# ajzhai/PEANUT

Hardware: AMD Instinct MI355X
Metric: maps/sec for 480x480x(4+N_cat) prediction fwd, batch 32 (higher is better)
Workload: dtype f32; 1 GPU; 480x480, 14-channel (4+10) partial maps -> 6-class prediction forward (PSPNet R50-V1c-D8), batch 32 per GPU, seeded random-init weights; survey_config=2, global_batch=32, parallelism=dp1 (map shards, no data-path collective)

## Files before the change

peanut_amd/csrc/conv_pw_ares.hip:

```cpp
#include <stdlib.h>

#include "common.h"
#include "conv_common.h"

namespace peanut {

namespace {

typedef const __attribute__((address_space(1))) void* gptr_t;
typedef __attribute__((address_space(3))) void* lptr_t;

__device__ __forceinline__ float load_uncounted(const float* ptr) {
  float v;
  asm volatile("global_load_dword %0, %1, off" : "=v"(v) : "v"(ptr) : "memory");
  return v;
}
template <int CH>
__device__ __forceinline__ void wait_uncounted(const float (&r)[CH], float a, float b) {
  static_assert(CH == 4 || CH == 8, "chunk of 4 or 8 values");
  __builtin_amdgcn_sched_barrier(0);
  if constexpr (CH == 4)
    asm volatile("s_waitcnt vmcnt(0)" ::"v"(r[0]), "v"(r[1]), "v"(r[2]), "v"(r[3]), "v"(a), "v"(b) : "memory");
  else
    asm volatile("s_waitcnt vmcnt(0)" ::"v"(r[0]), "v"(r[1]), "v"(r[2]), "v"(r[3]), "v"(r[4]), "v"(r[5]), "v"(r[6]), "v"(r[7]), "v"(a), "v"(b)
                 : "memory");
  __builtin_amdgcn_sched_barrier(0);
}

template <int NK, bool FLUSH>
__global__ __launch_bounds__(512) void conv_pw_ares_kernel(const ConvKParams p) {
  constexpr int BK = 32, K = NK * BK, TILE = 128 * BK;
  constexpr int CH = 32 / NK;
  static_assert(NK == 4 || NK == 8, "K = 128 or 256");
  __shared__ __attribute__((aligned(1024))) float smem[(NK + 2) * TILE];
  float* const bst = smem + NK * TILE;

  const int tid = threadIdx.x, lane = tid & 63;
  const int wave = __builtin_amdgcn_readfirstlane(tid >> 6);
  const int lr = lane >> 3, lp = lane & 7;
  const int wm = wave >> 2, wn = wave & 3;
  const int li = lane & 31, hi = lane >> 5;
  const bool late = p.phase_shift && wave >= 4;

  const int G = gridDim.x, bid = blockIdx.x;
  const int lw = (bid & 7) * (G >> 3) + (bid >> 3);
  const int NT = p.ntiles;
  const long long U = (long long)p.mtiles * NT;
  const int u0 = (int)(U * lw / G), u1 = (int)(U * (lw + 1) / G);
  if (u0 >= u1) return;

  const int pbn = p.ares_pbn;
  unsigned a_off[2], b_off[2];
#pragma unroll
  for (int j = 0; j < 2; ++j) {
    const int r = (wave * 2 + j) * 8 + lr;
    const int c = lp ^ ((r >> 1) & 7);
    a_off[j] = r * K + c * 4;
    b_off[j] = (r / pbn) * (NK * pbn * BK) + (r % pbn) * BK + c * 4;
  }
  auto dma_a = [&](int mt, int s) {
    const float* base = p.x + (size_t)mt * (128 * K) + s * BK;
#pragma unroll
    for (int j = 0; j < 2; ++j)
      __builtin_amdgcn_global_load_lds((gptr_t)(base + a_off[j]), (lptr_t)(smem + s * TILE + (wave * 2 + j) * 256), 16, 0, 0);
  };
  auto dma_b = [&](int mt, int nt, int kt, int stage) {
    const float* base = p.w + (p.mt_per_group ? (size_t)(mt / p.mt_per_group) * p.w_group_stride : 0) + (size_t)nt * (128 * K) + kt * (pbn * BK);
#pragma unroll
    for (int j = 0; j < 2; ++j)
      __builtin_amdgcn_global_load_lds((gptr_t)(base + b_off[j]), (lptr_t)(bst + stage * TILE + (wave * 2 + j) * 256), 16, 0, 0);
  };

  const int swz = (li >> 1) & 7;
  int sw[4];
#pragma unroll
  for (int ks = 0; ks < 4; ++ks) sw[ks] = ((ks * 2 + hi) ^ swz) * 4;
  const int a_row = (wm * 64 + li) * BK;
  const int b_row = (wn * 32 + li) * BK;

  f32x16 acc[2], acc2[2], prev[2];
#pragma unroll
  for (int t = 0; t < 2; ++t)
#pragma unroll
    for (int r = 0; r < 16; ++r) { acc[t][r] = 0.f; acc2[t][r] = 0.f; prev[t][r] = 0.f; }

  const size_t lane_el = (size_t)(wm * 64 + 4 * hi) * p.cout + wn * 32 + li;
  const bool has_res = p.res != nullptr;
  const size_t rstride = has_res ? (size_t)p.cout : 0;
  const size_t ostride = (size_t)p.cout;
  const float* res_run = has_res ? p.res + lane_el : p.zeros;
  float* out_run = p.y + lane_el;
  const float* prev_sc = p.scale + wn * 32 + li;
  const float* prev_sh = p.shift + wn * 32 + li;
  bool prev_valid = false;
  float scv = 1.f, shv = 0.f;
  const float alpha = p.alpha;
  const bool relu = p.relu != 0;

#define ARES_CHUNK_LOADS(kt)                                                              \
  float resv[CH];                                                                         \
  if ((kt) == 0) {                                                                        \
    scv = load_uncounted(prev_sc);                                                        \
    shv = load_uncounted(prev_sh);                                                        \
  }                                                                                       \
  _Pragma("unroll") for (int i = 0; i < CH; ++i)                                          \
    resv[i] = load_uncounted(res_run + (size_t)(8 * (i >> 2) + (i & 3)) * rstride);       \
  res_run += (size_t)(2 * CH) * rstride;
#define ARES_CHUNK_FINISH(kt)                                                             \
  if (prev_valid) {                                                   \
    _Pragma("unroll") for (int i = 0; i < CH; ++i) {                                      \
      const int idx = (kt) * CH + i;                                                      \
      float v = prev[idx >> 4][idx & 15] * (scv * alpha) + shv;                           \
      v += resv[i];                                                                       \
      if (relu) v = relu_keep_nan(v);                                                     \
      out_run[(size_t)(8 * (i >> 2) + (i & 3)) * ostride] = v;                            \
    }                                                                                     \
  }                                                                                       \
  out_run += (size_t)(2 * CH) * ostride;

  {
    const int mt = u0 / NT, nt = u0 - mt * NT;
#pragma unroll
    for (int s = 0; s < NK; ++s) dma_a(mt, s);
    dma_b(mt, nt, 0, 0);
    asm volatile("s_waitcnt vmcnt(0)" ::: "memory");
    __builtin_amdgcn_s_barrier();
    asm volatile("" ::: "memory");
  }

  int stage = 0;
  for (int u = u0; u < u1; ++u) {
    const int mt = u / NT, nt = u - mt * NT;
    const bool nxt = u + 1 < u1;
    const int mt_n = nxt ? (u + 1) / NT : mt;
    const int nt_n = nxt ? (u + 1) - mt_n * NT : 0;
    const bool refill_next = nxt && mt_n != mt;

    static_for<NK>([&](auto kc) {
      constexpr int kt = decltype(kc)::value;
      const float* const cur_b = bst + stage * TILE;
      const float* const cur_a = smem + kt * TILE;
      const bool more = (kt + 1 < NK) || nxt;
      ARES_CHUNK_LOADS(kt)
      auto request = [&]() {
        if (more) {
          if (kt + 1 < NK) dma_b(mt, nt, kt + 1, stage ^ 1);
          else dma_b(mt_n, nt_n, 0, stage ^ 1);
        }
      };
      if (!late) request();
      __builtin_amdgcn_sched_barrier(0);
      f32x4 af[4][2], bf[4];
#pragma unroll
      for (int j = 0; j < 4; ++j) {
        af[j][0] = *reinterpret_cast<const f32x4*>(cur_a + a_row + sw[j]);
        af[j][1] = *reinterpret_cast<const f32x4*>(cur_a + a_row + 32 * BK + sw[j]);
        bf[j] = *reinterpret_cast<const f32x4*>(cur_b + b_row + sw[j]);
      }
#pragma unroll
      for (int j = 0; j < 2; ++j)
#pragma unroll
        for (int kk = 0; kk < 4; ++kk)
#pragma unroll
          for (int t = 0; t < 2; ++t) acc[t] = __builtin_amdgcn_mfma_f32_32x32x2f32(af[j][t][kk], bf[j][kk], acc[t], 0, 0, 0);
      __builtin_amdgcn_sched_barrier(0);
      if (late) request();
      __builtin_amdgcn_sched_barrier(0);
#pragma unroll
      for (int j = 2; j < 4; ++j)
#pragma unroll
        for (int kk = 0; kk < 4; ++kk)
#pragma unroll
          for (int t = 0; t < 2; ++t) acc[t] = __builtin_amdgcn_mfma_f32_32x32x2f32(af[j][t][kk], bf[j][kk], acc[t], 0, 0, 0);
      if (FLUSH && (kt & 1)) {
#pragma unroll
        for (int t = 0; t < 2; ++t) {
          acc2[t] += acc[t];
#pragma unroll
          for (int r = 0; r < 16; ++r) acc[t][r] = 0.f;
        }
      }
      wait_uncounted<CH>(resv, scv, shv);
      ARES_CHUNK_FINISH(kt)
      if (kt >= 1) { if (refill_next) dma_a(mt_n, kt - 1); }
      asm volatile("s_waitcnt lgkmcnt(0)" ::: "memory");
      __builtin_amdgcn_s_barrier();
      asm volatile("" ::: "memory");
      stage ^= 1;
    });

#pragma unroll
    for (int t = 0; t < 2; ++t) {
      prev[t] = FLUSH ? acc2[t] : acc[t];
#pragma unroll
      for (int r = 0; r < 16; ++r) { acc[t][r] = 0.f; acc2[t][r] = 0.f; }
    }
    {
      const size_t unit_el = (size_t)mt * 128 * p.cout + (size_t)nt * 128 + lane_el;
      res_run = has_res ? p.res + unit_el : p.zeros;
      out_run = p.y + unit_el;
      const int ss_off = (p.mt_per_group && p.ss_group_stride) ? (mt / p.mt_per_group) * p.ss_group_stride : 0;
      prev_sc = p.scale + ss_off + nt * 128 + wn * 32 + li;
      prev_sh = p.shift + ss_off + nt * 128 + wn * 32 + li;
      prev_valid = true;
    }
    if (refill_next) dma_a(mt_n, NK - 1);
  }

  static_for<NK>([&](auto kc) {
    constexpr int kt = decltype(kc)::value;
    ARES_CHUNK_LOADS(kt)
    wait_uncounted<CH>(resv, scv, shv);
    ARES_CHUNK_FINISH(kt)
  });
#undef ARES_CHUNK_LOADS
#undef ARES_CHUNK_FINISH
}

template <int NK, bool FLUSH>
int launch_ares_t(ConvKParams p, hipStream_t stream) {
  const int cus = device_cus();
  if (cus < 8) return fail(-3, "conv_pw_ares: no current device");
  const long long U = (long long)p.mtiles * p.ntiles;
  long long G = U < cus ? U : cus;
  G -= G % 8;
  if (G < 8) return fail(-2, "conv_pw_ares: launch too small");
  hipLaunchKernelGGL((conv_pw_ares_kernel<NK, FLUSH>), dim3((unsigned)G), dim3(512), 0, stream, p);
  hipError_t e = hipGetLastError();
  if (e != hipSuccess) return fail(-3, std::string("conv_pw_ares launch: ") + hipGetErrorString(e));
  return 0;
}

}

bool conv_pw_uses_ares(int cin, int cout, long long M, int stride, bool two_source, int flush_ktiles, int bn_tile) {
  const bool on = opt(OPT_PW_ARES) != 0;
  const long long min_units = opt(OPT_PW_ARES_MINUNITS);
  if (!on || two_source || (cin != 128 && cin != 256) || stride != 1 || M % 128 != 0 || cout % 128 != 0) return false;
  if (bn_tile != 64 && bn_tile != 128) return false;
  if (flush_ktiles != 0 && flush_ktiles != 2) return false;
  return (M / 128) * (cout / 128) >= min_units;
}

int launch_conv_pw_ares(const ConvKParams& p0, int bn_tile, hipStream_t stream) {
  ConvKParams p = p0;
  p.phase_shift = opt(OPT_PW256_PHASE) != 0;
  p.ares_pbn = bn_tile;
  p.mtiles = p.M / 128;
  p.ntiles = p.cout / 128;
  const bool flush = p.flush == 2;
  if (p.c1 == 256) return flush ? launch_ares_t<8, true>(p, stream) : launch_ares_t<8, false>(p, stream);
  return flush ? launch_ares_t<4, true>(p, stream) : launch_ares_t<4, false>(p, stream);
}

}
```

Before: 888.1 maps/s.

## Defer epilogue stores by one chunk and use SGPR-base addressing in pointwise conv

The fused pointwise-conv epilogue now keeps each chunk's results in registers and issues their global stores during the next chunk's DMA request. The wait then lets those stores stay in flight (vmcnt(N)) instead of draining all memory ops before the barrier. Residual and output addressing switches to a scalar base plus a 32-bit per-lane offset to cut 64-bit address arithmetic, and the A-tile refill is issued earlier. The change also adds peeled first and second units, optional trace and ablation macros, and an s_nop before each load, which adds code complexity and may overflow 32-bit offsets on large tensors.

```diff
diff --git a/peanut_amd/csrc/conv_pw_ares.hip b/peanut_amd/csrc/conv_pw_ares.hip
--- a/peanut_amd/csrc/conv_pw_ares.hip
+++ b/peanut_amd/csrc/conv_pw_ares.hip
@@ -10,19 +10,21 @@
 typedef const __attribute__((address_space(1))) void* gptr_t;
 typedef __attribute__((address_space(3))) void* lptr_t;
 
-__device__ __forceinline__ float load_uncounted(const float* ptr) {
+__device__ __forceinline__ float load_uncounted(const float* base, unsigned byte_off) {
   float v;
-  asm volatile("global_load_dword %0, %1, off" : "=v"(v) : "v"(ptr) : "memory");
+  asm volatile("s_nop 4\n\tglobal_load_dword %0, %1, %2" : "=v"(v) : "v"(byte_off), "s"(base) : "memory");
   return v;
 }
-template <int CH>
+template <int CH, int N>
 __device__ __forceinline__ void wait_uncounted(const float (&r)[CH], float a, float b) {
   static_assert(CH == 4 || CH == 8, "chunk of 4 or 8 values");
+  static_assert(N == 0 || N == CH, "nothing, or the stores of one chunk");
   __builtin_amdgcn_sched_barrier(0);
   if constexpr (CH == 4)
-    asm volatile("s_waitcnt vmcnt(0)" ::"v"(r[0]), "v"(r[1]), "v"(r[2]), "v"(r[3]), "v"(a), "v"(b) : "memory");
+    asm volatile("s_waitcnt vmcnt(%0)" ::"n"(N), "v"(r[0]), "v"(r[1]), "v"(r[2]), "v"(r[3]), "v"(a), "v"(b) : "memory");
   else
-    asm volatile("s_waitcnt vmcnt(0)" ::"v"(r[0]), "v"(r[1]), "v"(r[2]), "v"(r[3]), "v"(r[4]), "v"(r[5]), "v"(r[6]), "v"(r[7]), "v"(a), "v"(b)
+    asm volatile("s_waitcnt vmcnt(%0)" ::"n"(N), "v"(r[0]), "v"(r[1]), "v"(r[2]), "v"(r[3]), "v"(r[4]), "v"(r[5]), "v"(r[6]), "v"(r[7]), "v"(a),
+                 "v"(b)
                  : "memory");
   __builtin_amdgcn_sched_barrier(0);
 }
@@ -84,39 +86,50 @@
 #pragma unroll
     for (int r = 0; r < 16; ++r) { acc[t][r] = 0.f; acc2[t][r] = 0.f; prev[t][r] = 0.f; }
 
-  const size_t lane_el = (size_t)(wm * 64 + 4 * hi) * p.cout + wn * 32 + li;
+  const unsigned lane_el = (unsigned)(wm * 64 + 4 * hi) * p.cout + wn * 32 + li;
   const bool has_res = p.res != nullptr;
-  const size_t rstride = has_res ? (size_t)p.cout : 0;
-  const size_t ostride = (size_t)p.cout;
-  const float* res_run = has_res ? p.res + lane_el : p.zeros;
-  float* out_run = p.y + lane_el;
-  const float* prev_sc = p.scale + wn * 32 + li;
-  const float* prev_sh = p.shift + wn * 32 + li;
-  bool prev_valid = false;
+  const unsigned rstride = has_res ? (unsigned)p.cout * 4u : 0u;
+  const unsigned ostride = (unsigned)p.cout * 4u;
+  const float* res_base = has_res ? p.res : p.zeros;
+  unsigned res_off = has_res ? lane_el * 4u : 0u;
+  float* out_base = p.y;
+  unsigned out_off = lane_el * 4u;
+  const unsigned ss_lane = (unsigned)(wn * 32 + li) * 4u;
   float scv = 1.f, shv = 0.f;
   const float alpha = p.alpha;
   const bool relu = p.relu != 0;
-
-#define ARES_CHUNK_LOADS(kt)                                                              \
+  float held[CH];
+  auto unit_el = [&](int u) {
+    const int mt = u / NT, nt = u - mt * NT;
+    return (size_t)mt * 128 * p.cout + (size_t)nt * 128;
+  };
+  auto unit_ss = [&](int u) {
+    const int mt = u / NT, nt = u - mt * NT;
+    const int ss_off = (p.mt_per_group && p.ss_group_stride) ? (mt / p.mt_per_group) * p.ss_group_stride : 0;
+    return ss_off + nt * 128;
+  };
+
+#define ARES_CHUNK_LOADS(kt, ss)                                                          \
   float resv[CH];                                                                         \
   if ((kt) == 0) {                                                                        \
-    scv = load_uncounted(prev_sc);                                                        \
-    shv = load_uncounted(prev_sh);                                                        \
+    scv = load_uncounted(p.scale + (ss), ss_lane);                                        \
+    shv = load_uncounted(p.shift + (ss), ss_lane);                                        \
   }                                                                                       \
   _Pragma("unroll") for (int i = 0; i < CH; ++i)                                          \
-    resv[i] = load_uncounted(res_run + (size_t)(8 * (i >> 2) + (i & 3)) * rstride);       \
-  res_run += (size_t)(2 * CH) * rstride;
+    resv[i] = load_uncounted(res_base, res_off + (unsigned)(8 * (i >> 2) + (i & 3)) * rstride); \
+  res_off += (unsigned)(2 * CH) * rstride;
 #define ARES_CHUNK_FINISH(kt)                                                             \
-  if (prev_valid) {                                                   \
-    _Pragma("unroll") for (int i = 0; i < CH; ++i) {                                      \
-      const int idx = (kt) * CH + i;                                                      \
-      float v = prev[idx >> 4][idx & 15] * (scv * alpha) + shv;                           \
-      v += resv[i];                                                                       \
-      if (relu) v = relu_keep_nan(v);                                                     \
-      out_run[(size_t)(8 * (i >> 2) + (i & 3)) * ostride] = v;                            \
-    }                                                                                     \
-  }                                                                                       \
-  out_run += (size_t)(2 * CH) * ostride;
+  _Pragma("unroll") for (int i = 0; i < CH; ++i) {                                        \
+    const int idx = (kt) * CH + i;                                                        \
+    float v = prev[idx >> 4][idx & 15] * (scv * alpha) + shv;                             \
+    v += resv[i];                                                                         \
+    if (relu) v = relu_keep_nan(v);                                                       \
+    held[i] = v;                                                                          \
+  }
+#define ARES_STORE_HELD()                                                                 \
+  _Pragma("unroll") for (int i = 0; i < CH; ++i)                                          \
+    *reinterpret_cast<float*>(reinterpret_cast<char*>(out_base) + (out_off + (unsigned)(8 * (i >> 2) + (i & 3)) * ostride)) = held[i]; \
+  out_off += (unsigned)(2 * CH) * ostride;
 
   {
     const int mt = u0 / NT, nt = u0 - mt * NT;
@@ -128,25 +141,60 @@
     asm volatile("" ::: "memory");
   }
 
+#ifdef PEANUT_ARES_TRACE
+  long long* const trace = reinterpret_cast<long long*>(p.partial) + blockIdx.x * 1024;
+  int trace_n = 0;
+#define ARES_TRACE(kind)                                                                                      \
+  if (blockIdx.x < 16 && tid == 0) {                                                                          \
+    ++trace_n;                                                                                                \
+    if (trace_n < 1024) trace[trace_n] = (long long)(__builtin_amdgcn_s_memtime() << 2) | (kind);             \
+    trace[0] = trace_n;                                                                                       \
+  }
+#else
+#define ARES_TRACE(kind)
+#endif
+#ifndef PEANUT_ARES_ABL
+#define PEANUT_ARES_ABL 0
+#endif
+
   int stage = 0;
-  for (int u = u0; u < u1; ++u) {
+  auto run_unit = [&](const int u, auto vc) {
+    constexpr int V = decltype(vc)::value;
     const int mt = u / NT, nt = u - mt * NT;
     const bool nxt = u + 1 < u1;
     const int mt_n = nxt ? (u + 1) / NT : mt;
     const int nt_n = nxt ? (u + 1) - mt_n * NT : 0;
     const bool refill_next = nxt && mt_n != mt;
+    const bool refill_last = V > 0 && (u - 1) / NT != mt;
+    const int ss = unit_ss(V > 0 ? u - 1 : u);
+    if (V > 0) {
+      if (has_res) res_base = p.res + unit_el(u - 1);
+      res_off = has_res ? lane_el * 4u : 0u;
+    }
+    asm volatile("" : "+v"(res_off));
 
     static_for<NK>([&](auto kc) {
       constexpr int kt = decltype(kc)::value;
+      constexpr bool STORES = !(PEANUT_ARES_ABL & 1) && (V == 2 || (V == 1 && kt >= 1));
       const float* const cur_b = bst + stage * TILE;
       const float* const cur_a = smem + kt * TILE;
-      const bool more = (kt + 1 < NK) || nxt;
-      ARES_CHUNK_LOADS(kt)
+      const bool more = !(PEANUT_ARES_ABL & 2) && ((kt + 1 < NK) || nxt);
+      ARES_CHUNK_LOADS(kt, ss)
+      if (kt >= 1) { if (refill_next) dma_a(mt_n, kt - 1); }
+      else { if (refill_last) dma_a(mt, NK - 1); }
       auto request = [&]() {
         if (more) {
           if (kt + 1 < NK) dma_b(mt, nt, kt + 1, stage ^ 1);
           else dma_b(mt_n, nt_n, 0, stage ^ 1);
         }
+        __builtin_amdgcn_sched_barrier(0);
+        if constexpr (STORES) { ARES_STORE_HELD() }
+        else if constexpr ((PEANUT_ARES_ABL & 1) != 0) { if (p.pad) { ARES_STORE_HELD() } }
+        if constexpr (V > 0 && kt == 0) {
+          out_base = p.y + unit_el(u - 1);
+          out_off = lane_el * 4u;
+          asm volatile("" : "+v"(out_off));
+        }
       };
       if (!late) request();
       __builtin_amdgcn_sched_barrier(0);
@@ -180,11 +228,11 @@
           for (int r = 0; r < 16; ++r) acc[t][r] = 0.f;
         }
       }
-      wait_uncounted<CH>(resv, scv, shv);
-      ARES_CHUNK_FINISH(kt)
-      if (kt >= 1) { if (refill_next) dma_a(mt_n, kt - 1); }
+      wait_uncounted<CH, STORES ? CH : 0>(resv, scv, shv);
+      ARES_TRACE(kt == 0 ? 0 : (refill_next ? 2 : 1))
+      if constexpr (V > 0) { ARES_CHUNK_FINISH(kt) }
       asm volatile("s_waitcnt lgkmcnt(0)" ::: "memory");
-      __builtin_amdgcn_s_barrier();
+      if constexpr (!(PEANUT_ARES_ABL & 4)) __builtin_amdgcn_s_barrier();
       asm volatile("" ::: "memory");
       stage ^= 1;
     });
@@ -195,26 +243,34 @@
 #pragma unroll
       for (int r = 0; r < 16; ++r) { acc[t][r] = 0.f; acc2[t][r] = 0.f; }
     }
-    {
-      const size_t unit_el = (size_t)mt * 128 * p.cout + (size_t)nt * 128 + lane_el;
-      res_run = has_res ? p.res + unit_el : p.zeros;
-      out_run = p.y + unit_el;
-      const int ss_off = (p.mt_per_group && p.ss_group_stride) ? (mt / p.mt_per_group) * p.ss_group_stride : 0;
-      prev_sc = p.scale + ss_off + nt * 128 + wn * 32 + li;
-      prev_sh = p.shift + ss_off + nt * 128 + wn * 32 + li;
-      prev_valid = true;
-    }
-    if (refill_next) dma_a(mt_n, NK - 1);
-  }
-
-  static_for<NK>([&](auto kc) {
-    constexpr int kt = decltype(kc)::value;
-    ARES_CHUNK_LOADS(kt)
-    wait_uncounted<CH>(resv, scv, shv);
-    ARES_CHUNK_FINISH(kt)
-  });
+  };
+  {
+    int u = u0;
+    run_unit(u++, IC<0>{});
+    if (u < u1) run_unit(u++, IC<1>{});
+    for (; u < u1; ++u) run_unit(u, IC<2>{});
+  }
+
+  if (!(PEANUT_ARES_ABL & 1) || p.pad) {
+    if (u1 - u0 >= 2) { ARES_STORE_HELD() }
+    out_base = p.y + unit_el(u1 - 1);
+    out_off = lane_el * 4u;
+    if (has_res) res_base = p.res + unit_el(u1 - 1);
+    res_off = has_res ? lane_el * 4u : 0u;
+    const int ss = unit_ss(u1 - 1);
+    static_for<NK>([&](auto kc) {
+      constexpr int kt = decltype(kc)::value;
+      ARES_CHUNK_LOADS(kt, ss)
+      wait_uncounted<CH, 0>(resv, scv, shv);
+      ARES_CHUNK_FINISH(kt)
+      ARES_STORE_HELD()
+    });
+  }
+  asm volatile("s_waitcnt vmcnt(0)" ::: "memory");
 #undef ARES_CHUNK_LOADS
 #undef ARES_CHUNK_FINISH
+#undef ARES_STORE_HELD
+#undef ARES_TRACE
 }
 
 template <int NK, bool FLUSH>
```

Measured after the change: 899.8 maps/s, median of 6. 1.01x the previous value.
